# cmitash/PhysimGlobalPose

Hardware: AMD Instinct MI355X
Metric: pose hypotheses/sec LCP-scored (50k-pt scene x 5k-pt model) (higher is better)
Workload: dtype f32

## Files before the change

### physimglobalpose_amd/csrc/lcp_score.hip

```cpp

#include "pgp_internal.h"

#include <hip/hip_ext.h>

#include <algorithm>
#include <cmath>
#include <cstdlib>
#include <cstring>
#include <vector>

namespace pgp {

namespace {

constexpr int kTile = 256;
constexpr int kMaxHpb = 64;

struct Xf {
  float m00, m10, m20, m01, m11, m21, m02, m12, m22, m03, m13, m23;
};

__device__ __forceinline__ Xf load_xf(const float* __restrict__ T, uint32_t h) {
  const float4* c = reinterpret_cast<const float4*>(T + 16u * h);
  float4 c0 = c[0], c1 = c[1], c2 = c[2], c3 = c[3];
// ... 861 lines not shown
        ebest = __uint_as_float((unsigned)(rest >> 32));
      }
      if (ebi >= 0) {
        bi = ebi;
        bs = ebest;
      }
    }
  }
  if (threadIdx.x == 0) {
    best[0] = bi;
    best[1] = (int)__float_as_uint(bs);
  }
}

struct HostPub {
  float* scores;
  int* counts;
  int* best;
  unsigned int* flag;
  unsigned int flag_value;
};

__device__ __forceinline__ const ScoreArgs& score_args_in_kernarg() {
#if defined(__HIP_DEVICE_COMPILE__)
  const ScoreArgs* ap = (const ScoreArgs*)__builtin_amdgcn_kernarg_segment_ptr();
  asm volatile("" : "+s"(ap));
  return *ap;
#else
  static const ScoreArgs none{};
  return none;
#endif
}

__global__ __launch_bounds__(256) void finalize_scores(ScoreArgs , const uint2* __restrict__ partial,
                                                       int n_tiles, int n_h, int nQ, int mode, int refine,
                                                       float* scores, int* __restrict__ counts,
                                                       unsigned long long* best_key, unsigned long long* runner_key,
                                                       unsigned int* ticket, int* __restrict__ best,
                                                       float* __restrict__ seq, HostPub hp) {
  int h = blockIdx.x * blockDim.x + threadIdx.x;
  unsigned long long key = 0;
  if (h < n_h) {
    int c = 0;
    float f = 0.f;
    constexpr int kFinTiles = 20;
    const uint4* p4 = reinterpret_cast<const uint4*>(partial);
    const int n_rows = nQ > 0 ? (nQ + 63) >> 6 : 1;
    const int last_pair = 2 * n_tiles - 1;
    for (int t0 = 0; t0 < n_tiles; t0 += kFinTiles) {
      uint4 pp[2 * kFinTiles];
#pragma unroll
      for (int j = 0; j < 2 * kFinTiles; ++j) pp[j] = p4[(size_t)min(2 * t0 + j, last_pair) * n_h + h];
#pragma unroll
      for (int j = 0; j < kFinTiles; ++j) {
        const int r0 = 4 * (t0 + j);
        if (r0 < n_rows) {
          const uint4 u = pp[2 * j], v = pp[2 * j + 1];
          const bool e1 = r0 + 1 < n_rows, e2 = r0 + 2 < n_rows, e3 = r0 + 3 < n_rows;
          c += (int)u.x + (e1 ? (int)u.z : 0) + (e2 ? (int)v.x : 0) + (e3 ? (int)v.z : 0);
          float ft = 0.f;
          ft += __uint_as_float(u.y);
          ft += e1 ? __uint_as_float(u.w) : 0.f;
          ft += e2 ? __uint_as_float(v.y) : 0.f;
          ft += e3 ? __uint_as_float(v.w) : 0.f;
          f += ft;
        }
      }
    }
    float score = (mode == PGP_MODE_PLAIN) ? __fdiv_rn((float)c, (float)nQ) : __fdiv_rn(f, (float)nQ);
    __hip_atomic_store(&scores[h], score, __ATOMIC_RELAXED, __HIP_MEMORY_SCOPE_AGENT);
    if (counts) counts[h] = c;
    if (hp.scores) {
      __hip_atomic_store(&hp.scores[h], score, __ATOMIC_RELAXED, __HIP_MEMORY_SCOPE_SYSTEM);
      __hip_atomic_store(&hp.counts[h], c, __ATOMIC_RELAXED, __HIP_MEMORY_SCOPE_SYSTEM);
    }
    if (score > 0.f)
      key = ((unsigned long long)__float_as_uint(score) << 32) | (unsigned long long)(0xFFFFFFFFu - (unsigned)h);
  }
  const unsigned long long mykey = key;
#pragma unroll
  for (int off = 32; off >= 1; off >>= 1) {
    unsigned long long o = __shfl_xor(key, off, 64);
    key = o > key ? o : key;
  }
  unsigned long long key2 = mykey == key ? 0ull : mykey;
#pragma unroll
  for (int off = 32; off >= 1; off >>= 1) {
    unsigned long long o = __shfl_xor(key2, off, 64);
    key2 = o > key2 ? o : key2;
  }
  __shared__ unsigned long long s_key[4], s_key2[4];
  __shared__ unsigned long long s_kk, s_kk2;
  __shared__ int s_last;
  if ((threadIdx.x & 63) == 0) {
    s_key[threadIdx.x >> 6] = key;
    s_key2[threadIdx.x >> 6] = key2;
  }
  asm volatile("s_waitcnt vmcnt(0)" ::: "memory");
  __syncthreads();
  if (threadIdx.x == 0) {
    unsigned long long k = 0, k2 = 0;
    for (int w = 0; w < 4; ++w) {
// ... 381 lines not shown

int tiles_for(int nQ) { return nQ > 0 ? (nQ + kTile - 1) / kTile : 1; }

void gate_thresholds(float gate_deg, float* c_aligned_min, float* c_anti_max) {
  *c_aligned_min = 2.f;
  *c_anti_max = -2.f;
  if (!(gate_deg == gate_deg)) return;
  if (gate_pred(1.0f, gate_deg)) {
    int32_t lo = f2key(0.0f), hi = f2key(1.0f);
    if (gate_pred(0.0f, gate_deg)) {
      *c_aligned_min = 0.0f;
    } else {
      while (hi - lo > 1) {
        int32_t mid = lo + (hi - lo) / 2;
        if (gate_pred(key2f(mid), gate_deg)) hi = mid; else lo = mid;
      }
      *c_aligned_min = key2f(hi);
    }
  }
  if (gate_pred(-1.0f, gate_deg)) {
    int32_t lo = f2key(-1.0f), hi = f2key(-0.0f);
    if (gate_pred(-0.0f, gate_deg)) {
      *c_anti_max = 0.0f;
    } else {
      while (hi - lo > 1) {
        int32_t mid = lo + (hi - lo) / 2;
        if (gate_pred(key2f(mid), gate_deg)) lo = mid; else hi = mid;
      }
      *c_anti_max = key2f(lo);
    }
  }
}

int launch_score(pgp_ctx* ctx, const float* d_T, int n_h, int mode, float gate_deg,
                 float* d_scores, int* d_counts, int* d_best, hipStream_t stream, ScoreHostOut* host) {
  ScoreArgs a{};
  if (host) host->published = false;
  int rc = await_index(ctx, stream);
  if (rc == PGP_OK) rc = nn_on_scoring_launch(ctx, stream);
  if (rc == PGP_OK) rc = fill_args(ctx, d_T, n_h, mode, gate_deg, stream, &a);
  if (rc != PGP_OK) return rc;
  if (n_h > ctx->cap_h) {
    set_error("n_h %d exceeds reserved capacity %d (pgp_reserve)", n_h, ctx->cap_h);
    return PGP_ESTATE;
  }
  unsigned long long* key = ctx->d_best.as<unsigned long long>();
  int* best_local = reinterpret_cast<int*>(key + 1);
  unsigned int* ticket = reinterpret_cast<unsigned int*>(key + 2);
  if (n_h > 0) {
    long long work = (long long)n_h * a.n_tiles;
    int hpb = ctx->hpb_override > 0 ? ctx->hpb_override : (int)(work / 10240);
    if (hpb < 4 && ctx->hpb_override <= 0) {
      hpb = (int)(work / 5120);
      hpb = hpb < 2 ? 2 : (hpb > 4 ? 4 : hpb);
    }
    if (ctx->hpb_override <= 0 && hpb > 16) hpb = 16;
    if (hpb > kMaxHpb) hpb = kMaxHpb;
    a.hpb = hpb;
    static const int tail_pct = getenv("PGP_TAIL_PCT") ? atoi(getenv("PGP_TAIL_PCT")) : 10;
    static const int tail_hpb = getenv("PGP_TAIL_HPB") ? atoi(getenv("PGP_TAIL_HPB")) : 2;
    a.hpb_tail = tail_hpb > 0 && tail_hpb <= hpb ? tail_hpb : hpb;
    int n_tail_h = (int)((long long)n_h * (tail_pct < 0 ? 0 : tail_pct > 100 ? 100 : tail_pct) / 100);
    a.n_big = (n_h - n_tail_h) / hpb;
    n_tail_h = n_h - a.n_big * hpb;
    a.n_chunks = a.n_big + (n_tail_h + a.hpb_tail - 1) / a.hpb_tail;
    a.partial = ctx->d_partial.as<uint2>();
    const long long n_blocks = (long long)((a.n_chunks + 7) / 8 * 8) * a.n_rows;
    if (n_blocks > 0x7FFFFFFFll) {
      set_error("scoring launch of %lld workgroups exceeds the grid limit", n_blocks);
      return PGP_EINVAL;
    }
    dim3 grid((unsigned)n_blocks);
    hipEvent_t ev0 = nullptr, ev1 = nullptr;
    if (ctx->timing > 0 && (ctx->timing_seq++ % (unsigned)ctx->timing) == 0) {
      if (ctx->ev_used + 2 > ctx->ev.size()) {
        for (int k = 0; k < 2; ++k) {
          hipEvent_t e;
          PGP_HIP(hipEventCreate(&e));
          ctx->ev.push_back(e);
        }
      }
      ev0 = ctx->ev[ctx->ev_used];
      ev1 = ctx->ev[ctx->ev_used + 1];
      ctx->ev_used += 2;
    }
    launch_variant(mode, ctx->unroll, grid, stream, a, ev0, ev1);
    hipLaunchKernelGGL(finalize_scores, dim3((n_h + 255) / 256), dim3(256), 0, stream, a,
                       (const uint2*)a.partial, a.n_tiles, n_h, a.nQ,
                       mode, ctx->refine_best ? 1 : 0, d_scores,
                       d_counts ? d_counts : (ctx->verify_early_out && mode == PGP_MODE_PLAIN ? ctx->d_counts.as<int>() : nullptr),
                       key, key + 3, ticket,
                       d_best ? d_best : best_local, ctx->d_seq.as<float>(),
                       host ? HostPub{host->scores, host->counts, host->best, host->flag, host->flag_value} : HostPub{});
    if (host) host->published = true;
  } else {
    hipLaunchKernelGGL(publish_none, dim3(1), dim3(1), 0, stream, d_best ? d_best : best_local);
  }
  PGP_HIP(hipGetLastError());
  if (ctx->exact_records && n_h > 0) return launch_settle_records(ctx, d_T, n_h, mode, gate_deg, d_scores, stream);
  if (ctx->verify_early_out && mode == PGP_MODE_PLAIN && n_h > 0)
    return launch_verify_early_out(ctx, d_T, n_h, d_scores, d_counts ? d_counts : ctx->d_counts.as<int>(), stream);
  return PGP_OK;
}

int launch_verify_early_out(pgp_ctx* ctx, const float* d_T, int n_h, float* d_scores, int* d_counts, hipStream_t stream) {
  if (n_h <= 0) return PGP_OK;
  ScoreArgs a{};
  int rc = await_index(ctx, stream);
  if (rc == PGP_OK) rc = fill_args(ctx, d_T, n_h, PGP_MODE_PLAIN, 30.f, stream, &a);
  if (rc != PGP_OK) return rc;
  if (ctx->d_eo_ws.cap < (size_t)n_h * sizeof(int) || !ctx->d_Qpos.p) {
    set_error("verify early-out: workspace not reserved (pgp_reserve / pgp_set_model)");
    return PGP_ESTATE;
  }
  int* tv = ctx->d_eo_ws.as<int>();
  hipLaunchKernelGGL(early_out_terminate_values, dim3(1), dim3(1024), 0, stream, (const int*)d_counts, n_h, a.nQ, tv);
  hipLaunchKernelGGL(early_out_walk, dim3((n_h + 3) / 4), dim3(256), 0, stream, a, (const int*)ctx->d_Qpos.as<int>(),
                     (const int*)tv, d_scores, d_counts);
  PGP_HIP(hipGetLastError());
// ... 139 lines not shown
```

### physimglobalpose_amd/csrc/multi_gpu.hip

```cpp

#include "pgp_internal.h"
#include "host_worker.h"

#include <rccl/rccl.h>

#include <dlfcn.h>
#include <fcntl.h>
#include <sys/mman.h>
#include <unistd.h>

#include <atomic>
#include <cerrno>
#include <chrono>
#include <condition_variable>
#include <cstdlib>
#include <cstring>
#include <functional>
#include <mutex>
#include <random>
#include <string>
#include <thread>
#include <vector>

namespace pgp {
// ... 22 lines not shown
  if (!r->handle) {
    set_error("RCCL not found (dlopen librccl.so.1): %s", dlerror());
    return false;
  }
#define PGP_SYM(field, name)                                             \
  r->field = reinterpret_cast<decltype(r->field)>(dlsym(r->handle, name)); \
  if (!r->field) {                                                       \
    set_error("RCCL symbol %s missing", name);                           \
    return false;                                                        \
  }
  PGP_SYM(CommInitAll, "ncclCommInitAll")
  PGP_SYM(CommInitRank, "ncclCommInitRank")
  PGP_SYM(GetUniqueId, "ncclGetUniqueId")
  PGP_SYM(CommCount, "ncclCommCount")
  PGP_SYM(CommDestroy, "ncclCommDestroy")
  PGP_SYM(AllReduce, "ncclAllReduce")
  PGP_SYM(GroupStart, "ncclGroupStart")
  PGP_SYM(GroupEnd, "ncclGroupEnd")
  PGP_SYM(GetErrorString, "ncclGetErrorString")
#undef PGP_SYM
  return true;
}


double now_ms() {
  return std::chrono::duration<double, std::milli>(std::chrono::steady_clock::now().time_since_epoch()).count();
}

}
}

using namespace pgp;

struct Streaming {
  hipStream_t x = nullptr;
  DevBuf ring[2];
  hipEvent_t scored[2] = {nullptr, nullptr}, reduced[2] = {nullptr, nullptr};
};
struct ShmExchange {
  struct Header {
    std::atomic<unsigned> arrived;
    unsigned pad[15];
  };
  Header* h = nullptr;
  unsigned char* data = nullptr;
  size_t cap = 0, total = 0;
  std::string name;
  unsigned seq = 0;
};
constexpr size_t kShmCap = (size_t)16 << 20;

constexpr int kSlots = 16;
constexpr int kEmulateMax = 16;

struct pgp_multi {
  int n = 0;
  int world = 0, rank0 = 0;
  long long n_exchanges = 0;
  std::vector<int> dev;
  std::vector<std::vector<pgp_ctx*>> octx;
  std::vector<hipStream_t> stream;
  std::vector<Worker*> worker;
  bool use_coll = false;
  bool emulate = false;
  bool emulate_ranked = false;
  ShmExchange shm;
  std::vector<hipEvent_t> ev;
  DevBuf d_sum;
  int fail[kEmulateMax] = {};
  Rccl rccl;
// ... 101 lines not shown

int shm_exchange(pgp_multi* m, float* d_s, int N, hipStream_t st) {
  ShmExchange& x = m->shm;
  const size_t bytes = (size_t)N * 8;
  if (bytes > x.cap) {
    set_error("PGP_MULTI_EMULATE_RANKED: %d hypotheses exceed the shared segment", N);
    return PGP_EINVAL;
  }
  int lo, hi;
  slice_of(N, m->rank0, m->world, &lo, &hi);
  unsigned char* buf = x.data + (size_t)(x.seq & 1u) * x.cap;
  if (hi > lo) {
    PGP_HIP(hipMemcpyAsync(buf + (size_t)lo * 4, d_s + lo, (size_t)(hi - lo) * 4, hipMemcpyDeviceToHost, st));
    PGP_HIP(hipMemcpyAsync(buf + (size_t)N * 4 + (size_t)lo * 4, reinterpret_cast<int*>(d_s + N) + lo, (size_t)(hi - lo) * 4,
                           hipMemcpyDeviceToHost, st));
  }
  PGP_HIP(hipStreamSynchronize(st));
  x.h->arrived.fetch_add(1u, std::memory_order_acq_rel);
  const unsigned want = (unsigned)m->world * (x.seq + 1u);
  const auto t_end = std::chrono::steady_clock::now() + std::chrono::seconds(120);
  while (x.h->arrived.load(std::memory_order_acquire) < want) {
    if (std::chrono::steady_clock::now() >= t_end) {
      set_error("PGP_MULTI_EMULATE_RANKED: a rank did not arrive at exchange %u", x.seq);
      return PGP_EHIP;
    }
    std::this_thread::yield();
  }
  PGP_HIP(hipMemcpyAsync(d_s, buf, bytes, hipMemcpyHostToDevice, st));
  PGP_HIP(hipStreamSynchronize(st));
  ++x.seq;
  return PGP_OK;
}

int score_piece(pgp_ctx* c, const float* d_T, int n, int mode, float gate_deg, float* d_scores, int* d_counts, int* d_best,
                hipStream_t st) {
  struct PassesOff {
    pgp_ctx* c;
    const bool records, early;
    explicit PassesOff(pgp_ctx* ctx) : c(ctx), records(ctx->exact_records), early(ctx->verify_early_out) {
      c->exact_records = false;
      c->verify_early_out = false;
    }
    ~PassesOff() {
      c->exact_records = records;
      c->verify_early_out = early;
    }
  } off(c);
  return pgp_score_lcp_device(c, d_T, n, mode, gate_deg, d_scores, d_counts, d_best, st);
}

struct Lane {
  int b;
  float* vec(pgp_multi* m, int j) const { return (b < 0 ? m->d_all[j] : m->s2[(size_t)j].ring[b]).as<float>(); }
  hipStream_t stream(pgp_multi* m, int j) const { return b < 0 ? m->stream[j] : m->s2[(size_t)j].x; }
  hipEvent_t queued(pgp_multi* m, int j) const { return b < 0 ? m->ev[j] : m->s2[(size_t)j].scored[b]; }
  hipEvent_t handed_out(pgp_multi* m) const { return b < 0 ? m->ev[0] : m->ev_sum[b]; }
};

int emulated_sum(pgp_multi* m, Lane lane, int N) {
  hipStream_t X = lane.stream(m, 0);
  SumPtrs ptrs{};
  for (int j = 0; j < m->n; ++j) {
    ptrs.p[j] = lane.vec(m, j);
    if (j > 0) PGP_HIP(hipStreamWaitEvent(X, lane.queued(m, j), 0));
  }
  float* d_out = m->d_sum.as<float>();
  hipLaunchKernelGGL(emulate_sum_args, dim3((2 * N + 255) / 256), dim3(256), 0, X, ptrs, m->n, N, d_out);
  PGP_HIP(hipGetLastError());
  for (int j = 0; j < m->n; ++j) PGP_HIP(hipMemcpyAsync(lane.vec(m, j), d_out, (size_t)N * 8, hipMemcpyDeviceToDevice, X));
  PGP_HIP(hipEventRecord(lane.handed_out(m), X));
  return PGP_OK;
}

int exchange(pgp_multi* m, int k, Lane lane, int N, int rc_slice) {
  hipStream_t S = m->stream[k], X = lane.stream(m, k);
  if (rc_slice == PGP_OK && (m->emulate || X != S)) {
    if (hipEventRecord(lane.queued(m, k), S) != hipSuccess) rc_slice = PGP_EHIP;
    if (rc_slice == PGP_OK && X != S && hipStreamWaitEvent(X, lane.queued(m, k), 0) != hipSuccess) rc_slice = PGP_EHIP;
  }
  int rc_x = PGP_OK;
  if (!m->emulate) {
    if (m->emulate_ranked) {
      rc_x = shm_exchange(m, lane.vec(m, k), N, X);
    } else {
      float* d_s = lane.vec(m, k);
      const ncclResult_t nr = m->rccl.AllReduce(d_s, d_s, 2 * (size_t)N, ncclInt32, ncclSum, m->comm[(size_t)k], X);
      if (nr != ncclSuccess) {
        set_error("ncclAllReduce failed: %s", m->rccl.GetErrorString(nr));
        rc_x = PGP_EHIP;
      }
    }
    return rc_slice != PGP_OK ? rc_slice : rc_x;
  }
  m->fail[k] = rc_slice != PGP_OK;
  m->barrier();
  bool any = false;
  for (int j = 0; j < m->n; ++j) any = any || m->fail[j];
  if (k == 0 && !any) {
    rc_x = emulated_sum(m, lane, N);
    m->fail[0] = rc_x != PGP_OK;
  }
  m->barrier();
  if (rc_slice != PGP_OK) return rc_slice;
  if (rc_x != PGP_OK) return rc_x;
  if (any || m->fail[0]) {
    set_error("another member of the group failed");
    return PGP_EHIP;
  }
  if (k > 0) PGP_HIP(hipStreamWaitEvent(X, lane.handed_out(m), 0));
  return PGP_OK;
}

// ... 8 lines not shown
}

void image_to_caller(const unsigned char* pin, int N, int n_obj, float* scores, int* counts, int* best_index, float* best_score) {
  if (N > 0) {
    if (scores) std::memcpy(scores, pin, (size_t)N * 4);
    if (counts) std::memcpy(counts, pin + (size_t)N * 4, (size_t)N * 4);
  }
  for (int o = 0; o < n_obj; ++o) {
    int best[2];
    std::memcpy(best, pin + (size_t)N * 8 + (size_t)o * 8, sizeof best);
    if (best_index) best_index[o] = best[0];
    if (best_score) std::memcpy(best_score + o, &best[1], 4);
  }
}

int score_flat(pgp_multi* m, int mode, float gate_deg, float* scores, int* counts, int* best_index, float* best_score) {
  const int N = m->total(), n_obj = (int)m->off.size() - 1;
  const double t0 = now_ms();
  int rc = m->h_pin.ensure((size_t)N * 72 + (size_t)n_obj * 8 + 256);
  if (rc != PGP_OK) return rc;
  unsigned char* pin_out = m->h_pin.as<unsigned char>() + (((size_t)N * 64 + 63) & ~(size_t)63);
  double t_enq = t0;

  auto score_slice = [&](int k) -> int {
    int lo, hi;
    slice_of(N, m->rank0 + k, m->world, &lo, &hi);
    float* d_s = m->d_all[k].as<float>();
    int* d_c = reinterpret_cast<int*>(d_s + N);
    if (N > 0 && m->world > 1) PGP_HIP(hipMemsetAsync(d_s, 0, (size_t)N * 8, m->stream[k]));
    for (int o = 0; o < n_obj; ++o) {
      const int a = std::max(lo, m->off[o]), b = std::min(hi, m->off[o + 1]);
      if (b <= a) continue;
      const int r = score_piece(m->octx[o][k], m->d_T[k].as<float>() + 16 * (size_t)a, b - a, mode, gate_deg, d_s + a, d_c + a,
                                nullptr, m->stream[k]);
      if (r != PGP_OK) return r;
    }
    return PGP_OK;
  };
  auto tail = [&]() -> int {
    float* d_s = m->d_all[0].as<float>();
    int* d_b = m->d_best[0].as<int>();
    hipStream_t st = m->stream[0];
    if (m->rest_pending) PGP_HIP(hipStreamWaitEvent(st, m->ev_rest, 0));
    for (int o = 0; o < n_obj; ++o) {
      const int a = m->off[o], cnt = m->off[o + 1] - a;
      const int r = complete_tail(m->octx[o][0], m->d_T[0].as<float>() + 16 * (size_t)a, cnt, mode, gate_deg, d_s + a,
                                  reinterpret_cast<int*>(d_s + N) + a, d_b + 2 * o, st, nullptr);
      if (r != PGP_OK) return r;
    }
    t_enq = now_ms();
    const PubItem items[2] = {{d_s, pin_out, (size_t)N * 8}, {d_b, pin_out + (size_t)N * 8, (size_t)n_obj * 8}};
    const PubItem* first = N > 0 ? items : items + 1;
    const int n_items = N > 0 ? 2 : 1;
    if (publish_usable(first, n_items)) return publish_and_wait(m->octx[0][0], st, first, n_items);
    if (N > 0) PGP_HIP(hipMemcpyAsync(pin_out, d_s, (size_t)N * 8, hipMemcpyDeviceToHost, st));
    PGP_HIP(hipMemcpyAsync(pin_out + (size_t)N * 8, d_b, (size_t)n_obj * 8, hipMemcpyDeviceToHost, st));
    PGP_HIP(hipStreamSynchronize(st));
    return PGP_OK;
  };
  const bool exchanging = m->exchange() && N > 0;
  if (exchanging) ++m->n_exchanges;
  rc = run_all(m, [&](int k) -> int {
    int r = score_slice(k);
    if (exchanging) r = exchange(m, k, Lane{-1}, N, r);
    return r == PGP_OK && k == 0 ? tail() : r;
  });
  if (rc != PGP_OK) return rc;
// ... 339 lines not shown
  if (workers) {
    run_all(m, [m](int k) -> int {
      if (m->stream[k]) (void)hipStreamSynchronize(m->stream[k]);
      if (k < (int)m->s2.size() && m->s2[(size_t)k].x) (void)hipStreamSynchronize(m->s2[(size_t)k].x);
      return PGP_OK;
    });
  }
  for (ncclComm_t c : m->comm)
    if (c) m->rccl.CommDestroy(c);
  if (workers) {
    run_all(m, [m](int k) -> int {
      m->d_T[k].release();
      m->d_all[k].release();
      m->d_best[k].release();
      if (k < (int)m->ev.size() && m->ev[k]) (void)hipEventDestroy(m->ev[k]);
      if (k == 0) {
        m->d_sum.release();
        m->d_best2.release();
        m->d_tail_seq.release();
        if (m->up_stream) {
          (void)hipStreamSynchronize(m->up_stream);
          (void)hipStreamDestroy(m->up_stream);
        }
        if (m->ev_rest) (void)hipEventDestroy(m->ev_rest);
        for (hipEvent_t ev : m->ev_sum)
          if (ev) (void)hipEventDestroy(ev);
      }
      if (k < (int)m->s2.size()) {
        Streaming& z = m->s2[(size_t)k];
        if (z.x) (void)hipStreamSynchronize(z.x);
        for (int b = 0; b < 2; ++b) {
          z.ring[b].release();
          if (z.scored[b]) (void)hipEventDestroy(z.scored[b]);
          if (z.reduced[b]) (void)hipEventDestroy(z.reduced[b]);
        }
        if (z.x) (void)hipStreamDestroy(z.x);
      }
      for (auto& per_slot : m->slot_T)
        if (k < (int)per_slot.size()) per_slot[(size_t)k].release();
      if (m->stream[k]) (void)hipStreamDestroy(m->stream[k]);
      for (auto& per_obj : m->octx)
        if (per_obj[(size_t)k]) pgp_destroy(per_obj[(size_t)k]);
      for (pgp_ctx* c : m->ictx[(size_t)k])
        if (c) pgp_destroy(c);
      return PGP_OK;
    });
  }
  for (Worker* w : m->worker) {
    w->shut_down();
    delete w;
  }
  if (m->shm.h) {
    (void)munmap(m->shm.h, m->shm.total);
    if (m->rank0 == 0) (void)shm_unlink(m->shm.name.c_str());
  }
  m->h_pin.release();
  delete m;
  return PGP_OK;
}

int pgp_multi_size(const pgp_multi* m) { return m ? m->n : 0; }

pgp_ctx* pgp_multi_context(pgp_multi* m, int k) { return (m && k >= 0 && k < m->n) ? m->octx[0][(size_t)k] : nullptr; }

int pgp_multi_add_object(pgp_multi* m) {
  if (!m) {
    set_error("pgp_multi_add_object: handle is NULL");
    return PGP_EINVAL;
// ... 120 lines not shown
  if (rc != PGP_OK) return rc;
  const float up = (float)(now_ms() - t0);
  rc = pgp_multi_score_uploaded(m, mode, gate_deg, scores, counts, best_index, best_score);
  m->last_ms[0] = up;
  return rc;
}

int pgp_multi_score_objects(pgp_multi* m, const float* const* T, const int* n_h, int n_obj, int mode, float gate_deg,
                            float* scores, int* counts, int* best_index, float* best_score) {
  if (!m || n_obj < 1 || !T || !n_h) {
    set_error("pgp_multi_score_objects: bad argument");
    return PGP_EINVAL;
  }
  const double t0 = now_ms();
  int rc = pgp_multi_upload_objects(m, T, n_h, n_obj);
  if (rc != PGP_OK) return rc;
  if (m->total() > 0 && !scores) {
    set_error("pgp_multi_score_objects: scores is NULL");
    return PGP_EINVAL;
  }
  const float up = (float)(now_ms() - t0);
  rc = score_flat(m, mode, gate_deg, scores, counts, best_index, best_score);
  m->last_ms[0] = up;
  return rc;
}

namespace {
int streaming_ready(pgp_multi* m, int k) {
  Streaming& z = m->s2[(size_t)k];
  if (z.x) return PGP_OK;
  PGP_HIP(hipStreamCreateWithFlags(&z.x, hipStreamNonBlocking));
  for (int b = 0; b < 2; ++b) {
    PGP_HIP(hipEventCreateWithFlags(&z.scored[b], hipEventDisableTiming));
    PGP_HIP(hipEventCreateWithFlags(&z.reduced[b], hipEventDisableTiming));
    if (k == 0 && m->emulate) PGP_HIP(hipEventCreateWithFlags(&m->ev_sum[b], hipEventDisableTiming));
  }
  if (k == 0) {
    const int r = m->d_best2.ensure(64);
    if (r != PGP_OK) return r;
  }
  return PGP_OK;
}

int queue_tail(pgp_multi* m, int b) {
  const int N = m->pend_n[b];
  if (N <= 0) return PGP_OK;
  float* d_s = m->s2[0].ring[b].as<float>();
  return complete_tail(m->octx[0][0], m->slot_T[(size_t)m->pend_slot[b]][0].as<float>(), N, m->pend_mode[b], m->pend_gate[b], d_s,
                       reinterpret_cast<int*>(d_s + N), m->d_best2.as<int>() + 2 * b, m->s2[0].x, m->d_tail_seq.as<float>());
}
}

int pgp_multi_upload_slot(pgp_multi* m, int slot, const float* T, int n_h) {
  if (!m || slot < 0 || slot >= kSlots || n_h < 0 || (n_h > 0 && !T) || n_h > 0x3FFFFFFF) {
    set_error("pgp_multi_upload_slot: bad argument (slot %d of %d, %d hypotheses)", slot, kSlots, n_h);
    return PGP_EINVAL;
  }
  if (m->step != 0) {
    set_error("pgp_multi_upload_slot: %lld steps are in flight (pgp_multi_collect first)", m->step);
    return PGP_ESTATE;
  }
  const int N = n_h;
  const size_t nT = (size_t)N * 64;
  int rc = m->h_pin.ensure(nT + (size_t)N * 8 + 256);
  if (rc != PGP_OK) return rc;
  if (nT) std::memcpy(m->h_pin.p, T, nT);
  rc = run_all(m, [m, slot, N, nT](int k) -> int {
    int lo, hi, r;
    slice_of(N, m->rank0 + k, m->world, &lo, &hi);
    if ((r = streaming_ready(m, k)) != PGP_OK) return r;
    Streaming& z = m->s2[(size_t)k];
    DevBuf& dT = m->slot_T[(size_t)slot][(size_t)k];
    if ((r = dT.ensure(nT + 64)) != PGP_OK) return r;
    for (int b = 0; b < 2; ++b)
      if ((r = z.ring[b].ensure((size_t)N * 8 + 64)) != PGP_OK) return r;
    if (k == 0 && m->emulate && (r = m->d_sum.ensure((size_t)N * 8 + 64)) != PGP_OK) return r;
    if (k == 0 && (r = m->d_tail_seq.ensure(std::max<size_t>(m->octx[0][0]->d_seq.cap, 64))) != PGP_OK) return r;
    if ((r = pgp_reserve(m->octx[0][(size_t)k], k == 0 ? N : hi - lo)) != PGP_OK) return r;
    const size_t a = k == 0 ? 0 : (size_t)lo * 64, b = k == 0 ? nT : (size_t)hi * 64;
    if (b > a)
      PGP_HIP(hipMemcpyAsync(dT.as<unsigned char>() + a, m->h_pin.as<unsigned char>() + a, b - a,
                             hipMemcpyHostToDevice, m->stream[k]));
    PGP_HIP(hipStreamSynchronize(m->stream[k]));
    return PGP_OK;
  });
  m->slot_n[(size_t)slot] = rc == PGP_OK ? N : -1;
  return rc;
}

int pgp_multi_enqueue_slot(pgp_multi* m, int slot, int mode, float gate_deg) {
  if (!m || slot < 0 || slot >= kSlots || m->slot_n[(size_t)slot] < 0) {
    set_error("pgp_multi_enqueue_slot: slot %d holds no batch (pgp_multi_upload_slot)", slot);
    return PGP_EINVAL;
  }
  const int N = m->slot_n[(size_t)slot];
  const int b = (int)(m->step & 1);
  const bool exchanging = m->exchange() && N > 0;
  m->pend_slot[b] = slot;
  m->pend_mode[b] = mode;
  m->pend_gate[b] = gate_deg;
  m->pend_n[b] = N;
  if (exchanging) ++m->n_exchanges;
  const long long step = m->step;
  const int rc = run_all(m, [&, m](int k) -> int {
    Streaming& z = m->s2[(size_t)k];
    hipStream_t S = m->stream[k], X = z.x;
    int lo, hi;
    slice_of(N, m->rank0 + k, m->world, &lo, &hi);
    float* d_s = z.ring[b].as<float>();
    int* d_c = reinterpret_cast<int*>(d_s + N);
    pgp_ctx* c = m->octx[0][(size_t)k];
    int r1 = [&]() -> int {
      if (!m->exchange())
        return pgp_score_lcp_device(c, m->slot_T[(size_t)slot][(size_t)k].as<float>(), N, mode, gate_deg, d_s, d_c,
                                    m->d_best2.as<int>() + 2 * b, S);
      if (step >= 2) PGP_HIP(hipStreamWaitEvent(S, z.reduced[b], 0));
      if (N > 0 && m->world > 1) PGP_HIP(hipMemsetAsync(d_s, 0, (size_t)N * 8, S));
      if (hi <= lo && N > 0) return PGP_OK;
      return score_piece(c, m->slot_T[(size_t)slot][(size_t)k].as<float>() + 16 * (size_t)lo, hi - lo, mode, gate_deg, d_s + lo,
                         d_c + lo, N == 0 && k == 0 ? m->d_best2.as<int>() + 2 * b : nullptr, S);
    }();
    if (!exchanging) return r1;
    r1 = exchange(m, k, Lane{b}, N, r1);
    if (r1 != PGP_OK) return r1;
    if (k == 0) {
      if (m->d_tail_seq.cap < c->d_seq.cap) {
        const int r = m->d_tail_seq.ensure(c->d_seq.cap);
        if (r != PGP_OK) return r;
      }
      const int r = queue_tail(m, b);
      if (r != PGP_OK) return r;
    }
    PGP_HIP(hipEventRecord(z.reduced[b], X));
    return PGP_OK;
  });
  if (rc != PGP_OK) return rc;
  ++m->step;
  return PGP_OK;
}

int pgp_multi_collect(pgp_multi* m, float* scores, int* counts, int* best_index, float* best_score) {
  if (!m) {
    set_error("pgp_multi_collect: handle is NULL");
    return PGP_EINVAL;
  }
  if (m->step == 0) {
    set_error("pgp_multi_collect: no step has been enqueued (pgp_multi_enqueue_slot)");
    return PGP_ESTATE;
  }
  const int b = (int)((m->step - 1) & 1);
  const int N = m->pend_n[b];
  unsigned char* pin_out = m->h_pin.as<unsigned char>();
  const int rc = run_all(m, [&, m](int k) -> int {
    Streaming& z = m->s2[(size_t)k];
    hipStream_t S = m->stream[k];
    PGP_HIP(hipStreamSynchronize(S));
    if (k == 0) {
      hipStream_t cs = m->exchange() && z.x ? z.x : S;
      if (N > 0) PGP_HIP(hipMemcpyAsync(pin_out, z.ring[b].p, (size_t)N * 8, hipMemcpyDeviceToHost, cs));
      PGP_HIP(hipMemcpyAsync(pin_out + (size_t)N * 8, m->d_best2.as<int>() + 2 * b, 8, hipMemcpyDeviceToHost, cs));
      if (cs == S) PGP_HIP(hipStreamSynchronize(S));
    }
    if (z.x) PGP_HIP(hipStreamSynchronize(z.x));
    return PGP_OK;
  });
  m->step = 0;
  if (rc != PGP_OK) return rc;
  image_to_caller(pin_out, N, 1, scores, counts, best_index, best_score);
  return PGP_OK;
}

int pgp_multi_last_timing(pgp_multi* m, float* upload_ms, float* enqueue_ms, float* total_ms) {
  if (!m) {
    set_error("pgp_multi_last_timing: handle is NULL");
    return PGP_EINVAL;
  }
  if (upload_ms) *upload_ms = m->last_ms[0];
  if (enqueue_ms) *enqueue_ms = m->last_ms[1];
  if (total_ms) *total_ms = m->last_ms[2];
  return PGP_OK;
}

int pgp_multi_icp_refine(pgp_multi* m, const pgp_multi_icp_job* jobs, int n_jobs, const pgp_icp_params* params) {
  if (!m || n_jobs < 0 || (n_jobs > 0 && !jobs) || !params) {
    set_error("pgp_multi_icp_refine: bad argument");
    return PGP_EINVAL;
  }
  std::vector<int> cnt((size_t)n_jobs, 0);
  for (int j = 0; j < n_jobs; ++j) {
    const pgp_multi_icp_job& q = jobs[j];
    if (q.n < 0 || q.n_src < 0 || q.n_tgt < 0 || (q.n > 0 && (!q.T || !q.src_xyz || !q.tgt_xyz || q.n_src == 0 || q.n_tgt == 0))) {
      set_error("pgp_multi_icp_refine: bad job %d", j);
      return PGP_EINVAL;
    }
    cnt[(size_t)j] = q.n;
  }
// ... 174 lines not shown
```

### physimglobalpose_amd/csrc/pgp_api.hip

```cpp

#include "pgp_internal.h"
#include "match_plan.h"

#include <chrono>

#include <algorithm>
#include <cfloat>
#include <cmath>
#include <cstdarg>
#include <cstdlib>
#include <cstring>
#include <numeric>
#include <vector>

namespace pgp {

static thread_local char g_err[512] = "";

void set_error(const char* fmt, ...) {
  va_list ap;
  va_start(ap, fmt);
  vsnprintf(g_err, sizeof g_err, fmt, ap);
  va_end(ap);
}
// ... 601 lines not shown
  const size_t n16 = bytes / 16;
  const int n_tail = (int)((bytes & 15u) / 4);
  hipLaunchKernelGGL(stage_from_host, dim3((unsigned)((n16 + (size_t)n_tail + 255) / 256)), dim3(256), 0, st,
                     static_cast<const uint4*>(h_pinned), static_cast<uint4*>(d_dst), n16, n_tail);
  PGP_HIP(hipGetLastError());
  return PGP_OK;
}
}

extern "C" {

int pgp_reserve(pgp_ctx* ctx, int max_hypotheses) {
  if (!ctx || max_hypotheses < 0) {
    set_error("pgp_reserve: bad argument");
    return PGP_EINVAL;
  }
  return reserve_impl(ctx, max_hypotheses);
}

static int reserve_impl(pgp_ctx* ctx, int max_hypotheses) {
  CtxGuard guard(ctx);
  if (int rc = flush_deferred_build(ctx)) return rc;
  if (ctx->index_pending && hipEventQuery(ctx->ev_index) == hipSuccess) {
    const int rc = finish_index(ctx);
    if (rc != PGP_OK) return rc;
  } else if (ctx->index_pending) {
    (void)hipGetLastError();
  }
  if (max_hypotheses <= ctx->cap_h) return PGP_OK;
  PGP_HIP(hipDeviceSynchronize());
  if (int rc = index_settled(ctx)) return rc;
  int rc;
  size_t cap = (size_t)max_hypotheses;
  size_t tiles = (size_t)tiles_for(ctx->nQ);
  if ((rc = ctx->d_T.ensure(cap * 16 * sizeof(float))) != PGP_OK) return rc;
  if ((rc = ctx->d_partial.ensure(4 * tiles * cap * (sizeof(int) + sizeof(float)))) != PGP_OK) return rc;
  if ((rc = ctx->d_scores.ensure(cap * sizeof(float))) != PGP_OK) return rc;
  if ((rc = ctx->d_counts.ensure(cap * sizeof(int))) != PGP_OK) return rc;
  if ((rc = ctx->d_eo_ws.ensure(cap * sizeof(int) + 64)) != PGP_OK) return rc;
  ctx->cap_h = max_hypotheses;
  return PGP_OK;
}

int pgp_score_lcp_device(pgp_ctx* ctx, const float* d_T, int n_h, int mode, float gate_deg,
                         float* d_scores, int* d_counts, int* d_best, void* stream) {
  if (!ctx || n_h < 0 || (n_h > 0 && (!d_T || !d_scores))) {
    set_error("pgp_score_lcp_device: bad argument");
    return PGP_EINVAL;
  }
  CtxGuard guard(ctx, false);
  const int rc = launch_score(ctx, d_T, n_h, mode, gate_deg, d_scores, d_counts, d_best,
                              static_cast<hipStream_t>(stream));
  note_device_work(ctx, static_cast<hipStream_t>(stream));
  return rc;
}

int pgp_set_exact_ties(pgp_ctx* ctx, int on) {
  if (!ctx) {
    set_error("pgp_set_exact_ties: ctx is NULL");
    return PGP_EINVAL;
  }
  CtxGuard guard(ctx);
  ctx->exact_ties = on != 0;
  if (!ctx->exact_ties) ctx->kd_valid = false;
  return PGP_OK;
}

int pgp_set_nn_pruning(pgp_ctx* ctx, int mode) {
  if (!ctx || mode < 0 || mode > 2) {
// ... 3309 lines not shown
```

### physimglobalpose_amd/csrc/pgp_internal.h

```cpp
#pragma once

#include <hip/hip_runtime.h>
#include <array>
#include <cstdint>
#include <cstdio>
#include <cstring>
#include <functional>
#include <string>
#include <vector>

#include "../../include/pgp.h"

namespace pgp {

void set_error(const char* fmt, ...);

#define PGP_HIP(call)                                                                   \
  do {                                                                                  \
    hipError_t _e = (call);                                                             \
    if (_e != hipSuccess) {                                                             \
      pgp::set_error("%s failed: %s (%s:%d)", #call, hipGetErrorString(_e), __FILE__, __LINE__); \
      return PGP_EHIP;                                                                  \
    }                                                                                   \
  } while (0)
// ... 404 lines not shown
                                const int* h_rows , int nb, float threshold, int* h_n_quads, hipStream_t st);
int launch_find_congruent_batch_lists(pgp_ctx* ctx, const float* h_base_xyz, const float* h_inv, const int* h_lists, int nb,
                                      float threshold, int* h_n_quads, hipStream_t st);
int launch_congruent_batch_gather(pgp_ctx* ctx, const int* h_picks, int m, int4* d_quads, hipStream_t st,
                                  const int2* d_picks_there = nullptr);
const uint32_t* congruent_batch_starts_device(pgp_ctx* ctx);

int launch_tetrahedron_bases(pgp_ctx* ctx, unsigned long long seed, int n_attempts, int triangle_trials, int fourth_trials,
                             float max_base_diameter, int* h_ids, float* h_dist, int* h_status, hipStream_t st);
int launch_v4pcs_join(pgp_ctx* ctx, const float* h_dist, int nb, float eps, long long cap, int4* d_quads, long long* h_counts,
                      hipStream_t st);
int launch_v4pcs_batch(pgp_ctx* ctx, const float* h_dist, int nb, float eps, int per_base_cap, long long* h_n_quads, int* h_n_stored,
                       hipStream_t st);
int launch_v4pcs_gather(pgp_ctx* ctx, const int* h_picks, int m, int4* d_out, hipStream_t st);

int launch_wide_bases(pgp_ctx* ctx, unsigned long long seed, int n_attempts, int triangle_trials, float max_base_diameter,
                      int* h_ids, float* h_inv, float* h_dist, int* h_status, float* h_xyz , hipStream_t st);
int launch_extract_pairs_batch(pgp_ctx* ctx, const float* h_dist, int nl, float eps, int* h_n_pairs, hipStream_t st);
int launch_extract_pairs_batch_gated(pgp_ctx* ctx, const float* h_dist, const int* h_base_ids, int nl, float eps,
                                     const pgp_pair_gates* gates, int* h_n_pairs, hipStream_t st);
int extract_pairs_batch_fetch(pgp_ctx* ctx, int list, int* h_pairs, int cap, int* h_n_pairs, hipStream_t st);

int tiles_for(int nQ);
struct ScoreHostOut {
  float* scores;
  int* counts;
  int* best;
  unsigned int* flag;
  unsigned int flag_value;
  bool published;
};
int launch_score(pgp_ctx* ctx, const float* d_T, int n_h, int mode, float gate_deg,
                 float* d_scores, int* d_counts, int* d_best, hipStream_t stream, ScoreHostOut* host = nullptr);
int launch_settle_best(pgp_ctx* ctx, const float* d_T, int n_h, int mode, float gate_deg, float* d_scores,
                       int* d_best, hipStream_t stream, float* seq_ws = nullptr);
int await_index(pgp_ctx* ctx, hipStream_t stream);
int finish_index(pgp_ctx* ctx);
int nn_on_scoring_launch(pgp_ctx* ctx, hipStream_t stream);
void nn_lists(pgp_ctx* ctx, hipStream_t stream, const uint2** occ_run, const float4** cand);
void nn_reset(pgp_ctx* ctx);
void nn_destroy(pgp_ctx* ctx);
int launch_settle_records(pgp_ctx* ctx, const float* d_T, int n_h, int mode, float gate_deg, float* d_scores,
                          hipStream_t stream);
int launch_verify_early_out(pgp_ctx* ctx, const float* d_T, int n_h, float* d_scores, int* d_counts, hipStream_t stream);
int records_workspace_bytes(int nQ);
int launch_registered_model(pgp_ctx* ctx, const float* d_T16, const float4* d_q, const float4* d_qn, int n,
                            float gate_deg, int* d_hits, hipStream_t stream);
int launch_registered(pgp_ctx* ctx, const float* d_T16, int mode, float gate_deg, int* d_hits,
                      hipStream_t stream);
void gate_thresholds(float gate_deg, float* c_aligned_min, float* c_anti_max);
int launch_count_neighbours(pgp_ctx* ctx, float radius, int* d_counts, hipStream_t stream);

int launch_select_top(pgp_ctx* ctx, const float* d_T, const float* d_scores, int n, int k, int invert, float* d_T_out,
                      int* d_idx_out, int* d_n_out, hipStream_t st);
struct IcpJob {
  pgp_ctx* ctx;
  const float4* d_src;
  int n_src;
  const float4* d_tgt;
  int n_tgt;
  float* d_T;
  int n;
  float* d_energy;
  int* d_iters;
  unsigned long long token;
};
// ... 127 lines not shown
```

Baseline: 50.41 million.

## Split scoring into partials and sum kernels pipelined across streams with partial ring

In the multi-GPU streaming path, scoring is split into a partial-tile kernel on the main stream and a separate sum_partials kernel on the exchange stream. Partial buffers rotate through a ring of up to eight slots, so the next batch's scoring can overlap the previous batch's reduction, exchange and tail. Synchronisation moves from per-step reduced events to summed events, waited on only periodically. This adds memory for the ring and more complex cross-stream ordering, and the periodic wait condition carries a risk of buffer-reuse hazards.

```diff
diff --git a/physimglobalpose_amd/csrc/lcp_score.hip b/physimglobalpose_amd/csrc/lcp_score.hip
--- a/physimglobalpose_amd/csrc/lcp_score.hip
+++ b/physimglobalpose_amd/csrc/lcp_score.hip
@@ -917,6 +917,48 @@
 #endif
 }
 
+template <int BATCH>
+__device__ __forceinline__ float score_of_partials(const uint2* __restrict__ partial, int n_tiles, int n_h, int nQ, int mode, int h,
+                                                   int* count) {
+  int c = 0;
+  float f = 0.f;
+  const uint4* p4 = reinterpret_cast<const uint4*>(partial);
+  const int n_rows = nQ > 0 ? (nQ + 63) >> 6 : 1;
+  const int last_pair = 2 * n_tiles - 1;
+  for (int t0 = 0; t0 < n_tiles; t0 += BATCH) {
+    uint4 pp[2 * BATCH];
+#pragma unroll
+    for (int j = 0; j < 2 * BATCH; ++j) pp[j] = p4[(size_t)min(2 * t0 + j, last_pair) * n_h + h];
+#pragma unroll
+    for (int j = 0; j < BATCH; ++j) {
+      const int r0 = 4 * (t0 + j);
+      if (r0 < n_rows) {
+        const uint4 u = pp[2 * j], v = pp[2 * j + 1];
+        const bool e1 = r0 + 1 < n_rows, e2 = r0 + 2 < n_rows, e3 = r0 + 3 < n_rows;
+        c += (int)u.x + (e1 ? (int)u.z : 0) + (e2 ? (int)v.x : 0) + (e3 ? (int)v.z : 0);
+        float ft = 0.f;
+        ft += __uint_as_float(u.y);
+        ft += e1 ? __uint_as_float(u.w) : 0.f;
+        ft += e2 ? __uint_as_float(v.y) : 0.f;
+        ft += e3 ? __uint_as_float(v.w) : 0.f;
+        f += ft;
+      }
+    }
+  }
+  *count = c;
+  return (mode == PGP_MODE_PLAIN) ? __fdiv_rn((float)c, (float)nQ) : __fdiv_rn(f, (float)nQ);
+}
+
+constexpr int kSumTiles = 4;
+__global__ __launch_bounds__(64) void sum_partials(const uint2* __restrict__ partial, int n_tiles, int n_h, int nQ, int mode,
+                                                   float* __restrict__ scores, int* __restrict__ counts) {
+  const int h = blockIdx.x * 64 + threadIdx.x;
+  if (h >= n_h) return;
+  int c;
+  scores[h] = score_of_partials<kSumTiles>(partial, n_tiles, n_h, nQ, mode, h, &c);
+  counts[h] = c;
+}
+
 __global__ __launch_bounds__(256) void finalize_scores(ScoreArgs , const uint2* __restrict__ partial,
                                                        int n_tiles, int n_h, int nQ, int mode, int refine,
                                                        float* scores, int* __restrict__ counts,
@@ -926,33 +968,9 @@
   int h = blockIdx.x * blockDim.x + threadIdx.x;
   unsigned long long key = 0;
   if (h < n_h) {
-    int c = 0;
-    float f = 0.f;
     constexpr int kFinTiles = 20;
-    const uint4* p4 = reinterpret_cast<const uint4*>(partial);
-    const int n_rows = nQ > 0 ? (nQ + 63) >> 6 : 1;
-    const int last_pair = 2 * n_tiles - 1;
-    for (int t0 = 0; t0 < n_tiles; t0 += kFinTiles) {
-      uint4 pp[2 * kFinTiles];
-#pragma unroll
-      for (int j = 0; j < 2 * kFinTiles; ++j) pp[j] = p4[(size_t)min(2 * t0 + j, last_pair) * n_h + h];
-#pragma unroll
-      for (int j = 0; j < kFinTiles; ++j) {
-        const int r0 = 4 * (t0 + j);
-        if (r0 < n_rows) {
-          const uint4 u = pp[2 * j], v = pp[2 * j + 1];
-          const bool e1 = r0 + 1 < n_rows, e2 = r0 + 2 < n_rows, e3 = r0 + 3 < n_rows;
-          c += (int)u.x + (e1 ? (int)u.z : 0) + (e2 ? (int)v.x : 0) + (e3 ? (int)v.z : 0);
-          float ft = 0.f;
-          ft += __uint_as_float(u.y);
-          ft += e1 ? __uint_as_float(u.w) : 0.f;
-          ft += e2 ? __uint_as_float(v.y) : 0.f;
-          ft += e3 ? __uint_as_float(v.w) : 0.f;
-          f += ft;
-        }
-      }
-    }
-    float score = (mode == PGP_MODE_PLAIN) ? __fdiv_rn((float)c, (float)nQ) : __fdiv_rn(f, (float)nQ);
+    int c;
+    const float score = score_of_partials<kFinTiles>(partial, n_tiles, n_h, nQ, mode, h, &c);
     __hip_atomic_store(&scores[h], score, __ATOMIC_RELAXED, __HIP_MEMORY_SCOPE_AGENT);
     if (counts) counts[h] = c;
     if (hp.scores) {
@@ -1400,6 +1418,74 @@
   }
 }
 
+namespace {
+int queue_scoring(pgp_ctx* ctx, ScoreArgs& a, int mode, uint2* partial, hipStream_t stream, hipEvent_t done) {
+  const int n_h = a.n_h;
+  long long work = (long long)n_h * a.n_tiles;
+  int hpb = ctx->hpb_override > 0 ? ctx->hpb_override : (int)(work / 10240);
+  if (hpb < 4 && ctx->hpb_override <= 0) {
+    hpb = (int)(work / 5120);
+    hpb = hpb < 2 ? 2 : (hpb > 4 ? 4 : hpb);
+  }
+  if (ctx->hpb_override <= 0 && hpb > 16) hpb = 16;
+  if (hpb > kMaxHpb) hpb = kMaxHpb;
+  a.hpb = hpb;
+  static const int tail_pct = getenv("PGP_TAIL_PCT") ? atoi(getenv("PGP_TAIL_PCT")) : 10;
+  static const int tail_hpb = getenv("PGP_TAIL_HPB") ? atoi(getenv("PGP_TAIL_HPB")) : 2;
+  a.hpb_tail = tail_hpb > 0 && tail_hpb <= hpb ? tail_hpb : hpb;
+  int n_tail_h = (int)((long long)n_h * (tail_pct < 0 ? 0 : tail_pct > 100 ? 100 : tail_pct) / 100);
+  a.n_big = (n_h - n_tail_h) / hpb;
+  n_tail_h = n_h - a.n_big * hpb;
+  a.n_chunks = a.n_big + (n_tail_h + a.hpb_tail - 1) / a.hpb_tail;
+  a.partial = partial;
+  const long long n_blocks = (long long)((a.n_chunks + 7) / 8 * 8) * a.n_rows;
+  if (n_blocks > 0x7FFFFFFFll) {
+    set_error("scoring launch of %lld workgroups exceeds the grid limit", n_blocks);
+    return PGP_EINVAL;
+  }
+  dim3 grid((unsigned)n_blocks);
+  hipEvent_t ev0 = nullptr, ev1 = nullptr;
+  if (ctx->timing > 0 && (ctx->timing_seq++ % (unsigned)ctx->timing) == 0) {
+    if (ctx->ev_used + 2 > ctx->ev.size()) {
+      for (int k = 0; k < 2; ++k) {
+        hipEvent_t e;
+        PGP_HIP(hipEventCreate(&e));
+        ctx->ev.push_back(e);
+      }
+    }
+    ev0 = ctx->ev[ctx->ev_used];
+    ev1 = ctx->ev[ctx->ev_used + 1];
+    ctx->ev_used += 2;
+  }
+  const bool attach = done && !ev1;
+  launch_variant(mode, ctx->unroll, grid, stream, a, ev0, attach ? done : ev1);
+  PGP_HIP(hipGetLastError());
+  if (done && !attach) PGP_HIP(hipEventRecord(done, stream));
+  return PGP_OK;
+}
+}
+
+size_t score_partial_bytes(const pgp_ctx* ctx, int n_h) {
+  return 4 * (size_t)tiles_for(ctx->nQ) * (size_t)(n_h > 0 ? n_h : 0) * sizeof(uint2);
+}
+
+int launch_score_partials(pgp_ctx* ctx, const float* d_T, int n_h, int mode, float gate_deg, void* d_partial, hipStream_t stream,
+                          hipEvent_t done) {
+  ScoreArgs a{};
+  int rc = await_index(ctx, stream);
+  if (rc == PGP_OK) rc = nn_on_scoring_launch(ctx, stream);
+  if (rc == PGP_OK) rc = fill_args(ctx, d_T, n_h, mode, gate_deg, stream, &a);
+  if (rc != PGP_OK) return rc;
+  return queue_scoring(ctx, a, mode, static_cast<uint2*>(d_partial), stream, done);
+}
+
+int launch_sum_partials(pgp_ctx* ctx, const void* d_partial, int n_h, int mode, float* d_scores, int* d_counts, hipStream_t stream) {
+  hipLaunchKernelGGL(sum_partials, dim3((n_h + 63) / 64), dim3(64), 0, stream, static_cast<const uint2*>(d_partial),
+                     tiles_for(ctx->nQ), n_h, ctx->nQ, mode, d_scores, d_counts);
+  PGP_HIP(hipGetLastError());
+  return PGP_OK;
+}
+
 int launch_score(pgp_ctx* ctx, const float* d_T, int n_h, int mode, float gate_deg,
                  float* d_scores, int* d_counts, int* d_best, hipStream_t stream, ScoreHostOut* host) {
   ScoreArgs a{};
@@ -1416,43 +1502,7 @@
   int* best_local = reinterpret_cast<int*>(key + 1);
   unsigned int* ticket = reinterpret_cast<unsigned int*>(key + 2);
   if (n_h > 0) {
-    long long work = (long long)n_h * a.n_tiles;
-    int hpb = ctx->hpb_override > 0 ? ctx->hpb_override : (int)(work / 10240);
-    if (hpb < 4 && ctx->hpb_override <= 0) {
-      hpb = (int)(work / 5120);
-      hpb = hpb < 2 ? 2 : (hpb > 4 ? 4 : hpb);
-    }
-    if (ctx->hpb_override <= 0 && hpb > 16) hpb = 16;
-    if (hpb > kMaxHpb) hpb = kMaxHpb;
-    a.hpb = hpb;
-    static const int tail_pct = getenv("PGP_TAIL_PCT") ? atoi(getenv("PGP_TAIL_PCT")) : 10;
-    static const int tail_hpb = getenv("PGP_TAIL_HPB") ? atoi(getenv("PGP_TAIL_HPB")) : 2;
-    a.hpb_tail = tail_hpb > 0 && tail_hpb <= hpb ? tail_hpb : hpb;
-    int n_tail_h = (int)((long long)n_h * (tail_pct < 0 ? 0 : tail_pct > 100 ? 100 : tail_pct) / 100);
-    a.n_big = (n_h - n_tail_h) / hpb;
-    n_tail_h = n_h - a.n_big * hpb;
-    a.n_chunks = a.n_big + (n_tail_h + a.hpb_tail - 1) / a.hpb_tail;
-    a.partial = ctx->d_partial.as<uint2>();
-    const long long n_blocks = (long long)((a.n_chunks + 7) / 8 * 8) * a.n_rows;
-    if (n_blocks > 0x7FFFFFFFll) {
-      set_error("scoring launch of %lld workgroups exceeds the grid limit", n_blocks);
-      return PGP_EINVAL;
-    }
-    dim3 grid((unsigned)n_blocks);
-    hipEvent_t ev0 = nullptr, ev1 = nullptr;
-    if (ctx->timing > 0 && (ctx->timing_seq++ % (unsigned)ctx->timing) == 0) {
-      if (ctx->ev_used + 2 > ctx->ev.size()) {
-        for (int k = 0; k < 2; ++k) {
-          hipEvent_t e;
-          PGP_HIP(hipEventCreate(&e));
-          ctx->ev.push_back(e);
-        }
-      }
-      ev0 = ctx->ev[ctx->ev_used];
-      ev1 = ctx->ev[ctx->ev_used + 1];
-      ctx->ev_used += 2;
-    }
-    launch_variant(mode, ctx->unroll, grid, stream, a, ev0, ev1);
+    if ((rc = queue_scoring(ctx, a, mode, ctx->d_partial.as<uint2>(), stream, nullptr)) != PGP_OK) return rc;
     hipLaunchKernelGGL(finalize_scores, dim3((n_h + 255) / 256), dim3(256), 0, stream, a,
                        (const uint2*)a.partial, a.n_tiles, n_h, a.nQ,
                        mode, ctx->refine_best ? 1 : 0, d_scores,
diff --git a/physimglobalpose_amd/csrc/multi_gpu.hip b/physimglobalpose_amd/csrc/multi_gpu.hip
--- a/physimglobalpose_amd/csrc/multi_gpu.hip
+++ b/physimglobalpose_amd/csrc/multi_gpu.hip
@@ -78,10 +78,20 @@
 
 using namespace pgp;
 
+constexpr int kPartialDepth = 8;
+constexpr size_t kPartialBudget = (size_t)32 << 20;
 struct Streaming {
   hipStream_t x = nullptr;
-  DevBuf ring[2];
-  hipEvent_t scored[2] = {nullptr, nullptr}, reduced[2] = {nullptr, nullptr};
+  DevBuf partial[kPartialDepth], ring[2];
+  int depth = 2;
+  size_t partial_bytes = 0;
+  hipEvent_t scored[2] = {nullptr, nullptr}, summed[2] = {nullptr, nullptr};
+  int ensure_partials(size_t bytes) {
+    partial_bytes = std::max(partial_bytes, bytes);
+    for (int p = 0; p < depth; ++p)
+      if (int r = partial[p].ensure(partial_bytes)) return r;
+    return PGP_OK;
+  }
 };
 struct ShmExchange {
   struct Header {
@@ -249,8 +259,7 @@
   return PGP_OK;
 }
 
-int score_piece(pgp_ctx* c, const float* d_T, int n, int mode, float gate_deg, float* d_scores, int* d_counts, int* d_best,
-                hipStream_t st) {
+int score_piece(pgp_ctx* c, const float* d_T, int n, int mode, float gate_deg, float* d_scores, int* d_counts, hipStream_t st) {
   struct PassesOff {
     pgp_ctx* c;
     const bool records, early;
@@ -263,14 +272,14 @@
       c->verify_early_out = early;
     }
   } off(c);
-  return pgp_score_lcp_device(c, d_T, n, mode, gate_deg, d_scores, d_counts, d_best, st);
+  return pgp_score_lcp_device(c, d_T, n, mode, gate_deg, d_scores, d_counts, nullptr, st);
 }
 
 struct Lane {
   int b;
   float* vec(pgp_multi* m, int j) const { return (b < 0 ? m->d_all[j] : m->s2[(size_t)j].ring[b]).as<float>(); }
   hipStream_t stream(pgp_multi* m, int j) const { return b < 0 ? m->stream[j] : m->s2[(size_t)j].x; }
-  hipEvent_t queued(pgp_multi* m, int j) const { return b < 0 ? m->ev[j] : m->s2[(size_t)j].scored[b]; }
+  hipEvent_t queued(pgp_multi* m, int j) const { return b < 0 ? m->ev[j] : m->s2[(size_t)j].summed[b]; }
   hipEvent_t handed_out(pgp_multi* m) const { return b < 0 ? m->ev[0] : m->ev_sum[b]; }
 };
 
@@ -291,10 +300,7 @@
 
 int exchange(pgp_multi* m, int k, Lane lane, int N, int rc_slice) {
   hipStream_t S = m->stream[k], X = lane.stream(m, k);
-  if (rc_slice == PGP_OK && (m->emulate || X != S)) {
-    if (hipEventRecord(lane.queued(m, k), S) != hipSuccess) rc_slice = PGP_EHIP;
-    if (rc_slice == PGP_OK && X != S && hipStreamWaitEvent(X, lane.queued(m, k), 0) != hipSuccess) rc_slice = PGP_EHIP;
-  }
+  if (rc_slice == PGP_OK && m->emulate && lane.b < 0 && hipEventRecord(lane.queued(m, k), S) != hipSuccess) rc_slice = PGP_EHIP;
   int rc_x = PGP_OK;
   if (!m->emulate) {
     if (m->emulate_ranked) {
@@ -369,7 +375,7 @@
       const int a = std::max(lo, m->off[o]), b = std::min(hi, m->off[o + 1]);
       if (b <= a) continue;
       const int r = score_piece(m->octx[o][k], m->d_T[k].as<float>() + 16 * (size_t)a, b - a, mode, gate_deg, d_s + a, d_c + a,
-                                nullptr, m->stream[k]);
+                                m->stream[k]);
       if (r != PGP_OK) return r;
     }
     return PGP_OK;
@@ -775,8 +781,9 @@
         for (int b = 0; b < 2; ++b) {
           z.ring[b].release();
           if (z.scored[b]) (void)hipEventDestroy(z.scored[b]);
-          if (z.reduced[b]) (void)hipEventDestroy(z.reduced[b]);
+          if (z.summed[b]) (void)hipEventDestroy(z.summed[b]);
         }
+        for (DevBuf& p : z.partial) p.release();
         if (z.x) (void)hipStreamDestroy(z.x);
       }
       for (auto& per_slot : m->slot_T)
@@ -963,7 +970,7 @@
   PGP_HIP(hipStreamCreateWithFlags(&z.x, hipStreamNonBlocking));
   for (int b = 0; b < 2; ++b) {
     PGP_HIP(hipEventCreateWithFlags(&z.scored[b], hipEventDisableTiming));
-    PGP_HIP(hipEventCreateWithFlags(&z.reduced[b], hipEventDisableTiming));
+    PGP_HIP(hipEventCreateWithFlags(&z.summed[b], hipEventDisableTiming));
     if (k == 0 && m->emulate) PGP_HIP(hipEventCreateWithFlags(&m->ev_sum[b], hipEventDisableTiming));
   }
   if (k == 0) {
@@ -975,7 +982,6 @@
 
 int queue_tail(pgp_multi* m, int b) {
   const int N = m->pend_n[b];
-  if (N <= 0) return PGP_OK;
   float* d_s = m->s2[0].ring[b].as<float>();
   return complete_tail(m->octx[0][0], m->slot_T[(size_t)m->pend_slot[b]][0].as<float>(), N, m->pend_mode[b], m->pend_gate[b], d_s,
                        reinterpret_cast<int*>(d_s + N), m->d_best2.as<int>() + 2 * b, m->s2[0].x, m->d_tail_seq.as<float>());
@@ -1005,6 +1011,9 @@
     if ((r = dT.ensure(nT + 64)) != PGP_OK) return r;
     for (int b = 0; b < 2; ++b)
       if ((r = z.ring[b].ensure((size_t)N * 8 + 64)) != PGP_OK) return r;
+    z.partial_bytes = std::max(z.partial_bytes, score_partial_bytes(m->octx[0][(size_t)k], hi - lo) + 64);
+    z.depth = (int)std::min<size_t>(kPartialDepth, std::max<size_t>(2, kPartialBudget / z.partial_bytes));
+    if ((r = z.ensure_partials(z.partial_bytes)) != PGP_OK) return r;
     if (k == 0 && m->emulate && (r = m->d_sum.ensure((size_t)N * 8 + 64)) != PGP_OK) return r;
     if (k == 0 && (r = m->d_tail_seq.ensure(std::max<size_t>(m->octx[0][0]->d_seq.cap, 64))) != PGP_OK) return r;
     if ((r = pgp_reserve(m->octx[0][(size_t)k], k == 0 ? N : hi - lo)) != PGP_OK) return r;
@@ -1042,28 +1051,32 @@
     int* d_c = reinterpret_cast<int*>(d_s + N);
     pgp_ctx* c = m->octx[0][(size_t)k];
     int r1 = [&]() -> int {
-      if (!m->exchange())
-        return pgp_score_lcp_device(c, m->slot_T[(size_t)slot][(size_t)k].as<float>(), N, mode, gate_deg, d_s, d_c,
-                                    m->d_best2.as<int>() + 2 * b, S);
-      if (step >= 2) PGP_HIP(hipStreamWaitEvent(S, z.reduced[b], 0));
-      if (N > 0 && m->world > 1) PGP_HIP(hipMemsetAsync(d_s, 0, (size_t)N * 8, S));
-      if (hi <= lo && N > 0) return PGP_OK;
-      return score_piece(c, m->slot_T[(size_t)slot][(size_t)k].as<float>() + 16 * (size_t)lo, hi - lo, mode, gate_deg, d_s + lo,
-                         d_c + lo, N == 0 && k == 0 ? m->d_best2.as<int>() + 2 * b : nullptr, S);
+      if (m->world > 1 && N > 0) PGP_HIP(hipMemsetAsync(d_s, 0, (size_t)N * 8, X));
+      if (hi > lo) {
+        const size_t need = score_partial_bytes(c, hi - lo);
+        if (z.partial_bytes < need) {
+          const int r = z.ensure_partials(need);
+          if (r != PGP_OK) return r;
+        }
+        DevBuf& part = z.partial[step % z.depth];
+        if (step >= 2 && step % (z.depth - 1) == 0) PGP_HIP(hipStreamWaitEvent(S, z.summed[b], 0));
+        int r = launch_score_partials(c, m->slot_T[(size_t)slot][(size_t)k].as<float>() + 16 * (size_t)lo, hi - lo, mode, gate_deg,
+                                      part.p, S, z.scored[b]);
+        c->device_work_pending = true;
+        if (r != PGP_OK) return r;
+        PGP_HIP(hipStreamWaitEvent(X, z.scored[b], 0));
+        if ((r = launch_sum_partials(c, part.p, hi - lo, mode, d_s + lo, d_c + lo, X)) != PGP_OK) return r;
+      }
+      PGP_HIP(hipEventRecord(z.summed[b], X));
+      return PGP_OK;
     }();
-    if (!exchanging) return r1;
-    r1 = exchange(m, k, Lane{b}, N, r1);
-    if (r1 != PGP_OK) return r1;
-    if (k == 0) {
-      if (m->d_tail_seq.cap < c->d_seq.cap) {
-        const int r = m->d_tail_seq.ensure(c->d_seq.cap);
-        if (r != PGP_OK) return r;
-      }
-      const int r = queue_tail(m, b);
+    if (exchanging) r1 = exchange(m, k, Lane{b}, N, r1);
+    if (r1 != PGP_OK || k != 0) return r1;
+    if (m->d_tail_seq.cap < c->d_seq.cap) {
+      const int r = m->d_tail_seq.ensure(c->d_seq.cap);
       if (r != PGP_OK) return r;
     }
-    PGP_HIP(hipEventRecord(z.reduced[b], X));
-    return PGP_OK;
+    return queue_tail(m, b);
   });
   if (rc != PGP_OK) return rc;
   ++m->step;
@@ -1084,15 +1097,12 @@
   unsigned char* pin_out = m->h_pin.as<unsigned char>();
   const int rc = run_all(m, [&, m](int k) -> int {
     Streaming& z = m->s2[(size_t)k];
-    hipStream_t S = m->stream[k];
-    PGP_HIP(hipStreamSynchronize(S));
+    PGP_HIP(hipStreamSynchronize(m->stream[k]));
     if (k == 0) {
-      hipStream_t cs = m->exchange() && z.x ? z.x : S;
-      if (N > 0) PGP_HIP(hipMemcpyAsync(pin_out, z.ring[b].p, (size_t)N * 8, hipMemcpyDeviceToHost, cs));
-      PGP_HIP(hipMemcpyAsync(pin_out + (size_t)N * 8, m->d_best2.as<int>() + 2 * b, 8, hipMemcpyDeviceToHost, cs));
-      if (cs == S) PGP_HIP(hipStreamSynchronize(S));
-    }
-    if (z.x) PGP_HIP(hipStreamSynchronize(z.x));
+      if (N > 0) PGP_HIP(hipMemcpyAsync(pin_out, z.ring[b].p, (size_t)N * 8, hipMemcpyDeviceToHost, z.x));
+      PGP_HIP(hipMemcpyAsync(pin_out + (size_t)N * 8, m->d_best2.as<int>() + 2 * b, 8, hipMemcpyDeviceToHost, z.x));
+    }
+    PGP_HIP(hipStreamSynchronize(z.x));
     return PGP_OK;
   });
   m->step = 0;
diff --git a/physimglobalpose_amd/csrc/pgp_api.hip b/physimglobalpose_amd/csrc/pgp_api.hip
--- a/physimglobalpose_amd/csrc/pgp_api.hip
+++ b/physimglobalpose_amd/csrc/pgp_api.hip
@@ -657,9 +657,8 @@
   if (int rc = index_settled(ctx)) return rc;
   int rc;
   size_t cap = (size_t)max_hypotheses;
-  size_t tiles = (size_t)tiles_for(ctx->nQ);
   if ((rc = ctx->d_T.ensure(cap * 16 * sizeof(float))) != PGP_OK) return rc;
-  if ((rc = ctx->d_partial.ensure(4 * tiles * cap * (sizeof(int) + sizeof(float)))) != PGP_OK) return rc;
+  if ((rc = ctx->d_partial.ensure(score_partial_bytes(ctx, max_hypotheses))) != PGP_OK) return rc;
   if ((rc = ctx->d_scores.ensure(cap * sizeof(float))) != PGP_OK) return rc;
   if ((rc = ctx->d_counts.ensure(cap * sizeof(int))) != PGP_OK) return rc;
   if ((rc = ctx->d_eo_ws.ensure(cap * sizeof(int) + 64)) != PGP_OK) return rc;
diff --git a/physimglobalpose_amd/csrc/pgp_internal.h b/physimglobalpose_amd/csrc/pgp_internal.h
--- a/physimglobalpose_amd/csrc/pgp_internal.h
+++ b/physimglobalpose_amd/csrc/pgp_internal.h
@@ -460,6 +460,10 @@
 };
 int launch_score(pgp_ctx* ctx, const float* d_T, int n_h, int mode, float gate_deg,
                  float* d_scores, int* d_counts, int* d_best, hipStream_t stream, ScoreHostOut* host = nullptr);
+size_t score_partial_bytes(const pgp_ctx* ctx, int n_h);
+int launch_score_partials(pgp_ctx* ctx, const float* d_T, int n_h, int mode, float gate_deg, void* d_partial, hipStream_t stream,
+                          hipEvent_t done);
+int launch_sum_partials(pgp_ctx* ctx, const void* d_partial, int n_h, int mode, float* d_scores, int* d_counts, hipStream_t stream);
 int launch_settle_best(pgp_ctx* ctx, const float* d_T, int n_h, int mode, float gate_deg, float* d_scores,
                        int* d_best, hipStream_t stream, float* seq_ws = nullptr);
 int await_index(pgp_ctx* ctx, hipStream_t stream);
```

New measurement: 50.40 million, median of 3. About the same (-0.0%).
